# bobu36000/gym-chess

Hardware: AMD Instinct MI355X
Metric: env steps/sec at 65 536 boards per GPU (random-policy self-play to terminal, auto-reset) (higher is better)
Workload: dtype u64

## Files before the change

### gym-chess_amd/csrc/gc_host_env.h

```cpp
#pragma once

static bool srv_enabled() {
    static const bool off = getenv("GC_SINGLE_SERVER") && atoi(getenv("GC_SINGLE_SERVER")) == 0;
    return !off;
}
static int srv_stop(void* p) {
    gc_env* e = static_cast<gc_env*>(p);
    return e->srv.stop(e->device, e);
}
static int srv_call(gc_env* e, int board, int op, int action, int flags) {
    return e->srv.call(
        e->device, e, srv_stop,
        [&](SrvBox* b) {
            if (e->srv.launch && e->srv_board != board && (srv_stop(e) || devsrv_claim(devsrv(e->device), e, srv_stop)))
                return -1;
            __atomic_store_n(&b->op, (u32)op, __ATOMIC_RELAXED);
            __atomic_store_n(&b->action, action, __ATOMIC_RELAXED);
            __atomic_store_n(&b->flags, (u32)flags, __ATOMIC_RELAXED);
            return 0;
        },
        [&]() -> int {
            HIPCHK(hipStreamSynchronize(e->stream));
            e->srv_board = board;
            return 0;
        },
        [&](SrvBox* box_d, u32 seq, u32 launch) {
            k_single_server<<<1, 64, 0, e->srv.stream>>>(e->d, board, box_d, e->srec_d, seq, launch);
        });
}

static int set_window_kind(gc_env* e, bool uncapped) {
    const int bits = uncapped ? HTAB_BITS_UNCAPPED : HTAB_BITS;
    if (bits != e->d.hbits) {
        size_t nb64 = ((size_t)e->n + 63) / 64 * 64;
        u64* t = nullptr;
        if (dalloc(&t, ((size_t)8 << bits) * nb64)) return -1;
        HIPCHK(hipMemsetAsync(t, 0, ((size_t)64 << bits) * nb64, e->stream));
        (void)hipFree(e->d.htab);
        e->d.htab = t;
        e->d.hbits = bits;
    }
    if (uncapped && !e->d.ic.spill.ent) {
        if (spill_alloc(e, spill_bits_for(e->n))) return -1;
    } else if (!uncapped && e->d.ic.spill.ent) {
        HIPCHK(hipStreamSynchronize(e->stream));
        spill_drop(e);
        if (spill_publish(e)) return -1;
    }
    return 0;
}

static void launch_reset(gc_env* e, const uint8_t* mask, int select) {
    if (e->rules && e->d.opp) k_fenv_reset<true><<<grid_for(e->n), BLOCK, 0, e->stream>>>(e->d, mask, select);
    else if (e->rules) k_fenv_reset<false><<<grid_for(e->n), BLOCK, 0, e->stream>>>(e->d, mask, select);
    else if (e->d.opp) k_env_reset<true><<<grid_for(e->n), BLOCK, 0, e->stream>>>(e->d, mask, select);
    else k_env_reset<false><<<grid_for(e->n), BLOCK, 0, e->stream>>>(e->d, mask, select);
}
template <bool POLICY>
static void launch_step(gc_env* e) {
    if (e->rules && e->d.opp) k_fenv_step<POLICY, true><<<grid_for(e->n), BLOCK, 0, e->stream>>>(e->d);
    else if (e->rules) k_fenv_step<POLICY, false><<<grid_for(e->n), BLOCK, 0, e->stream>>>(e->d);
    else if (e->d.opp) k_env_step<POLICY, true><<<grid_for(e->n), BLOCK, 0, e->stream>>>(e->d);
    else k_env_step<POLICY, false><<<grid_for(e->n), BLOCK, 0, e->stream>>>(e->d);
}

struct ResetInfo {
    const EnvDev::InitCache* icd;
    const uint16_t* racts;
    u32 rinfo;
};
static ResetInfo reset_info(const gc_env* e) {
    const EnvDev::InitCache& ic = e->rules ? e->ic_f : e->d.ic;
    return ResetInfo{e->rules ? e->icd_f : e->icd, e->rules ? e->racts_f : e->d.reset_acts,
                     (ic.table ? 1u << 16 : 0u) | (u32)(ic.total & 0xFFFF)};
}

static const uint16_t* sw_table(const ResetInfo& r) {
    return r.racts ? r.racts + RESET_ACTS_MAX : r.racts;
}
static bool pair_ok(const gc_env* e) {
    if (!e->d.opp) return true;
    if (e->rules) return false;
    const EnvDev::InitCache& ic = e->d.ic;
    return ic.usable && ic.table && (!e->d.agent_black || ic.open_safe);
}
static int pair_opp(const gc_env* e) { return e->d.opp ? (e->d.agent_black ? 2 : 1) : 0; }

static_assert(PAIR_BOARDS == QUAD_BOARDS, "one board block size");
struct LaunchGeom {
    dim3 grid, block;
};
static int board_blocks(const gc_env* e) { return (e->n + PAIR_BOARDS - 1) / PAIR_BOARDS; }
static LaunchGeom pair_geom(int nb) { return {dim3((nb + PAIRS_WG - 1) / PAIRS_WG), dim3(2 * PAIR_BOARDS * PAIRS_WG)}; }
static LaunchGeom quad_geom(int nb) { return {dim3((nb + QUADS_WG - 1) / QUADS_WG), dim3(4 * QUAD_BOARDS * QUADS_WG)}; }

template <class K>
static K pair_variant(const gc_env* e, K fide, K none, K vs_white, K vs_black) {
    if (e->rules) return fide;
    const int opp = pair_opp(e);
    return opp == 0 ? none : opp == 1 ? vs_white : vs_black;
}
static const uint16_t* pair_racts(const gc_env* e, const ResetInfo& r) { return e->rules ? r.racts : sw_table(r); }

static void launch_step2(gc_env* e, hipStream_t st, int b0 = 0, int nb = -1) {
    const EnvDev& d = e->d;
    const ResetInfo r = reset_info(e);
    const LaunchGeom g = pair_geom(nb < 0 ? board_blocks(e) : nb);
    const auto kernel = pair_variant(e, k_env_step2<true>, k_env_step2<false>, k_env_step2<false, 1>, k_env_step2<false, 2>);
    kernel<<<g.grid, g.block, 0, st>>>(e->slab, d.n, b0, d.seed, d.htab, pair_racts(e, r), r.icd, r.rinfo);
}

extern "C" int gc_env_create(int device, int n_boards, uint64_t seed, const int8_t* initial_board, gc_env** out) {
    if (!out) return fail("null out pointer");
    if (n_boards <= 0) return fail("n_boards must be > 0");
    int nd = 0;
    HIPCHK(hipGetDeviceCount(&nd));
    if (device < 0 || device >= nd) return fail("device index out of range");
    static const int8_t DEF[64] = {-3, -5, -4, -2, -1, -4, -5, -3, -6, -6, -6, -6, -6, -6, -6, -6,
                                   0,  0,  0,  0,  0,  0,  0,  0,  0,  0,  0,  0,  0,  0,  0,  0,
                                   0,  0,  0,  0,  0,  0,  0,  0,  0,  0,  0,  0,  0,  0,  0,  0,
                                   6,  6,  6,  6,  6,  6,  6,  6,  3,  5,  4,  2,  1,  4,  5,  3};
    const int8_t* ib = initial_board ? initial_board : DEF;
    if (check_boards(1, ib)) return -1;
    gc_env* e = new gc_env();
    e->device = device;
    e->n = n_boards;
    e->seed = seed;
    int n = n_boards;
    size_t nb64 = ((size_t)n + 63) / 64 * 64;
    hipError_t he = hipSetDevice(device);
    if (he == hipSuccess) he = hipStreamCreateWithFlags(&e->stream, hipStreamNonBlocking);
    if (he != hipSuccess) { env_free(e); delete e; return fail(std::string("stream: ") + hipGetErrorString(he)); }
    if (dalloc(&e->slab, Slab::BYTES_PER_BOARD * (size_t)n) ||
        dalloc(&e->d.htab, (size_t)HTAB * 8 * nb64) || dalloc(&e->mbox, (size_t)64 * n) ||
        dalloc(&e->m8, (size_t)8 * n) || dalloc(&e->mask, n) || dalloc(&e->counts, n) || dalloc(&e->stats, (size_t)8 * n + 8) ) {
        std::string m = g_err;
        env_free(e); delete e;
        return fail(m);
    }
    {
        uint8_t* sl = e->slab;
        size_t nz = (size_t)n;
        e->bb = reinterpret_cast<u64*>(sl);
        e->meta = reinterpret_cast<u32*>(sl + Slab::meta(nz));
        e->d.hgen = reinterpret_cast<u32*>(sl + Slab::hgen(nz));
        e->d.draw = reinterpret_cast<u32*>(sl + Slab::draw(nz));
        e->d.nsteps = reinterpret_cast<u32*>(sl + Slab::nsteps(nz));
        e->d.reward = reinterpret_cast<int32_t*>(sl + Slab::reward(nz));
        e->d.act = reinterpret_cast<uint16_t*>(sl + Slab::act(nz));
        e->d.done = sl + Slab::done(nz);
        e->d.reason = sl + Slab::reason(nz);
    }
    Pos ip = from_mailbox(ib, 0);
    u64 ibb[NBB] = {ip.k, ip.q, ip.r, ip.b, ip.n, ip.p, ip.w};
    for (int j = 0; j < NBB; j++) e->d.init[j] = ibb[j];
    he = hipSuccess;
    if (he == hipSuccess) he = hipMemsetAsync(e->d.draw, 0, (size_t)4 * n, e->stream);
    if (he == hipSuccess) he = hipMemsetAsync(e->d.htab, 0, (size_t)64 * HTAB * nb64, e->stream);
    if (he == hipSuccess) he = hipMemsetAsync(e->d.hgen, 0, (size_t)4 * n, e->stream);
    if (he == hipSuccess) he = hipMemsetAsync(e->d.nsteps, 0, (size_t)4 * n, e->stream);
    if (he == hipSuccess) he = hipMemsetAsync(e->d.reward, 0, (size_t)4 * n, e->stream);
    if (he == hipSuccess) he = hipMemsetAsync(e->d.done, 0, (size_t)n, e->stream);
    if (he == hipSuccess) he = hipMemsetAsync(e->d.reason, 0, (size_t)n, e->stream);
    if (he == hipSuccess) he = hipMemsetAsync(e->stats, 0, (size_t)64 * n, e->stream);
    for (auto& v : e->ev) if (he == hipSuccess) he = hipEventCreate(&v);
    if (he != hipSuccess) { env_free(e); delete e; return fail(std::string("env init: ") + hipGetErrorString(he)); }
    e->d.st = SoA{e->bb, e->meta, n};
    e->d.seed = seed;
    e->d.n = n;
    e->d.opp = 0;
    e->d.agent_black = 0;
    e->d.hbits = HTAB_BITS;
    {
        EnvDev::InitCache* dic = nullptr;
        uint16_t* dacts = nullptr;
        if (dalloc(&dic, 1) || dalloc(&dacts, 2 * RESET_ACTS_MAX)) {
            std::string m = g_err; (void)hipFree(dic); env_free(e); delete e; return fail(m);
// ... 344 lines not shown
    if (kind < 0 || kind > 3) return fail("kind: 0 h2h, 1 h2d, 2 d2h, 3 d2d");
    HIPCHK(hipSetDevice(e->device));
    HIPCHK(hipMemcpyAsync(dst, src, bytes, (hipMemcpyKind)kind, e->stream));
    HIPCHK(hipStreamSynchronize(e->stream));
    return 0;
}

static int issue_plies(gc_env* e, int n) {
    if (e->n_sub <= 1) {
        for (int p = 0; p < n; p++) launch_step2(e, e->stream);
        HIPCHK(hipGetLastError());
        return 0;
    }
    const int blocks = board_blocks(e);
    const int k = e->n_sub < blocks ? e->n_sub : blocks;
    const int per = ((blocks + k - 1) / k + PAIRS_WG - 1) / PAIRS_WG * PAIRS_WG;
    HIPCHK(hipEventRecord(e->fork_ev, e->stream));
    for (int j = 0; j < k; j++) HIPCHK(hipStreamWaitEvent(e->sub[j], e->fork_ev, 0));
    for (int p = 0; p < n; p++)
        for (int j = 0; j < k; j++) {
            int b0 = j * per, nb = blocks - b0 < per ? blocks - b0 : per;
            if (nb > 0) launch_step2(e, e->sub[j], b0, nb);
        }
    HIPCHK(hipGetLastError());
    for (int j = 0; j < k; j++) {
        HIPCHK(hipEventRecord(e->sub_ev[j], e->sub[j]));
        HIPCHK(hipStreamWaitEvent(e->stream, e->sub_ev[j], 0));
    }
    return 0;
}

static int step_random(gc_env* e, int n_plies) {
    if (pair_ok(e)) return n_plies > 0 ? issue_plies(e, n_plies) : 0;
    for (int p = 0; p < n_plies; p++) {
        launch_step<true>(e);
        HIPCHK(hipGetLastError());
    }
    return 0;
}
extern "C" int gc_env_step_random(gc_env* e, int n_plies) {
    if (!e) return fail("null env");
    SRV_QUIESCE(e);
    if (!e->policy_ready) return fail("policy actions stale: call gc_env_reset or gc_env_select_random first");
    HIPCHK(hipSetDevice(e->device));
    if (spill_before(e)) return -1;
    for (int p = 0; p < n_plies;) {
        const int k = spill_chunk(e, n_plies - p);
        if (k < 0 || step_random(e, k)) return -1;
        p += k;
    }
    return spill_after(e);
}

extern "C" int gc_env_set_streams(gc_env* e, int k) {
    if (!e) return fail("null env");
    if (k < 1 || k > GC_MAX_SUBSTREAMS) return fail("streams must be in [1, 8]");
    HIPCHK(hipSetDevice(e->device));
    for (int j = 0; j < k; j++) {
        if (!e->sub[j]) HIPCHK(hipStreamCreateWithFlags(&e->sub[j], hipStreamNonBlocking));
        if (!e->sub_ev[j]) HIPCHK(hipEventCreateWithFlags(&e->sub_ev[j], hipEventDisableTiming));
    }
    if (!e->fork_ev) HIPCHK(hipEventCreateWithFlags(&e->fork_ev, hipEventDisableTiming));
    e->n_sub = k;
    return 0;
}

extern "C" int gc_env_paired(gc_env* e) {
    if (!e) return fail("null env");
    return pair_ok(e) ? 1 : 0;
}

static bool use_quad(const gc_env* e) {
    static const bool no_quad = getenv("GC_NO_QUAD") != nullptr;
    return !no_quad && !e->rules && pair_opp(e) == 0 && e->d.ic.table;
}

static int occ_min_plies() {
    static const int v = getenv("GC_OCC_MIN_PLIES") ? atoi(getenv("GC_OCC_MIN_PLIES")) : 600;
    return v;
}

extern "C" int gc_env_rollout_occ_min_plies(void) { return occ_min_plies(); }

extern "C" int gc_env_rollout_waves(gc_env* e) {
    if (!e) return fail("null env");
    return pair_ok(e) ? (use_quad(e) ? 4 : 2) : 1;
}

extern "C" int gc_env_select_random(gc_env* e) {
    if (!e) return fail("null env");
    SRV_QUIESCE(e);
    HIPCHK(hipSetDevice(e->device));
    if (e->rules) k_fenv_select<<<grid_for(e->n), BLOCK, 0, e->stream>>>(e->d);
    else k_select<<<grid_for(e->n), BLOCK, 0, e->stream>>>(e->d);
    HIPCHK(hipGetLastError());
    e->policy_ready = true;
    return 0;
}

static int issue_rollout(gc_env* e, int n_plies, uint64_t* d_trace, bool stats) {
    uint64_t* const st = stats ? e->stats : nullptr;
    const bool pair = pair_ok(e);
    const EnvDev& d = e->d;
    const ResetInfo r = reset_info(e);
    const LaunchGeom pg = pair_geom(board_blocks(e)), qg = quad_geom(board_blocks(e));
    for (int p0 = 0, k = 0; p0 < n_plies; p0 += k) {
        k = spill_chunk(e, n_plies - p0 < ROLLOUT_MAX_PLIES ? n_plies - p0 : ROLLOUT_MAX_PLIES);
        if (k < 0) return -1;
        u64* tr = d_trace ? reinterpret_cast<u64*>(d_trace) + (size_t)p0 * e->n : nullptr;
        const u32 ri = r.rinfo | ((u32)k << 18);
        e->done_expect = 0;
        if (pair && use_quad(e)) {
            const auto kernel = k >= occ_min_plies() ? k_env_rollout4<true> : k_env_rollout4<false>;
            kernel<<<qg.grid, qg.block, 0, e->stream>>>(e->slab, d.n, d.seed, d.htab, sw_table(r), r.icd, ri, st, tr);
            e->done_expect = ++e->done_issued;
        } else if (pair) {
            const auto kernel = pair_variant(e, k_env_rollout2<true>, k_env_rollout2<false>, k_env_rollout2<false, 1>,
                                             k_env_rollout2<false, 2>);
            kernel<<<pg.grid, pg.block, 0, e->stream>>>(e->slab, d.n, d.seed, d.htab, pair_racts(e, r), r.icd, ri, st, tr);
        } else if (e->rules) {
            k_fenv_rollout<true><<<grid_for(e->n), BLOCK, 0, e->stream>>>(e->d, k, tr, st);
        } else if (e->d.opp) {
            k_env_rollout<true><<<grid_for(e->n), BLOCK, 0, e->stream>>>(e->d, k, tr, st);
        } else {
            k_env_rollout<false><<<grid_for(e->n), BLOCK, 0, e->stream>>>(e->d, k, tr, st);
        }
        hipError_t le = hipGetLastError();
        if (le != hipSuccess) return fail(std::string("rollout launch: ") + hipGetErrorString(le));
    }
    return 0;
}

extern "C" int gc_env_rollout(gc_env* e, int n_plies, int16_t* tr_action, int16_t* tr_reward, uint8_t* tr_done,
                              uint8_t* tr_reason, uint64_t* stats8) {
    if (!e) return fail("null env");
    SRV_QUIESCE(e);
    if (n_plies < 0) return fail("n_plies must be >= 0");
    if (!e->policy_ready) return fail("policy actions stale: call gc_env_reset or gc_env_select_random first");
    HIPCHK(hipSetDevice(e->device));
    const bool trace = tr_action || tr_reward || tr_done || tr_reason;
    const size_t cnt = (size_t)n_plies * e->n;
    Temps tmps;
    u64* dt = nullptr;
    if (trace && cnt && tmps.alloc(&dt, cnt)) return -1;
    if (spill_before(e)) return -1;
    HIPCHK(hipMemsetAsync(e->stats, 0, (size_t)64 * e->n, e->stream));
    if (issue_rollout(e, n_plies, dt, true) || spill_after(e)) return -1;
    if (trace && cnt) {
        std::vector<u64> h(cnt);
        hipError_t ce = hipMemcpyAsync(h.data(), dt, cnt * 8, hipMemcpyDeviceToHost, e->stream);
        if (ce == hipSuccess) ce = hipStreamSynchronize(e->stream);
        if (ce != hipSuccess) return fail(std::string("rollout trace: ") + hipGetErrorString(ce));
        for (size_t t = 0; t < cnt; t++) {
            const u64 w = h[t];
            if (tr_action) tr_action[t] = (int16_t)(uint16_t)w;
            if (tr_reward) tr_reward[t] = (int16_t)(uint16_t)(w >> 16);
            if (tr_done) tr_done[t] = (uint8_t)(w >> 32);
            if (tr_reason) tr_reason[t] = (uint8_t)(w >> 40);
        }
    }
    if (stats8) {
        uint64_t* sums = e->stats + (size_t)8 * e->n;
        HIPCHK(hipMemsetAsync(sums, 0, 64, e->stream));
        k_sum_stats<<<grid_for(e->n), BLOCK, 0, e->stream>>>(e->stats, e->n, reinterpret_cast<unsigned long long*>(sums));
        HIPCHK(hipGetLastError());
        HIPCHK(hipMemcpyAsync(stats8, sums, 64, hipMemcpyDeviceToHost, e->stream));
        HIPCHK(hipStreamSynchronize(e->stream));
    }
    return 0;
}

extern "C" int gc_env_rollout_device(gc_env* e, int n_plies, uint64_t* d_trace, int ev_begin, int ev_end) {
    if (!e) return fail("null env");
    SRV_QUIESCE(e);
    if (n_plies < 0) return fail("n_plies must be >= 0");
    if (ev_begin < -1 || ev_begin >= 8 || ev_end < -1 || ev_end >= 8) return fail("event slots: -1 or 0..7");
    if (!e->policy_ready) return fail("policy actions stale: call gc_env_reset or gc_env_select_random first");
    HIPCHK(hipSetDevice(e->device));
    if (spill_before(e)) return -1;
    if (ev_begin >= 0) HIPCHK(hipEventRecord(e->ev[ev_begin], e->stream));
    if (issue_rollout(e, n_plies, d_trace, false)) return -1;
    if (ev_end >= 0) HIPCHK(hipEventRecord(e->ev[ev_end], e->stream));
    return spill_after(e);
}

extern "C" int gc_env_get_outputs(gc_env* e, int32_t* reward, uint8_t* done, uint8_t* reason, uint16_t* next_action,
                                  uint32_t* nsteps) {
    if (!e) return fail("null env");
    SRV_QUIESCE(e);
    HIPCHK(hipSetDevice(e->device));
    if (reward) HIPCHK(hipMemcpyAsync(reward, e->d.reward, (size_t)4 * e->n, hipMemcpyDeviceToHost, e->stream));
    if (done) HIPCHK(hipMemcpyAsync(done, e->d.done, e->n, hipMemcpyDeviceToHost, e->stream));
    if (reason) HIPCHK(hipMemcpyAsync(reason, e->d.reason, e->n, hipMemcpyDeviceToHost, e->stream));
    if (next_action) HIPCHK(hipMemcpyAsync(next_action, e->d.act, (size_t)2 * e->n, hipMemcpyDeviceToHost, e->stream));
    if (nsteps) HIPCHK(hipMemcpyAsync(nsteps, e->d.nsteps, (size_t)4 * e->n, hipMemcpyDeviceToHost, e->stream));
    HIPCHK(hipStreamSynchronize(e->stream));
// ... 83 lines not shown
    if (!e || !mask) return fail("null argument");
    SRV_QUIESCE(e);
    HIPCHK(hipSetDevice(e->device));
    if (!e->lmask && dalloc(&e->lmask, (size_t)65 * e->n)) return -1;
    if (e->rules) k_fmask<<<grid_for(e->n), BLOCK, 0, e->stream>>>(e->d.st, e->lmask, e->counts);
    else k_mask<<<grid_for(e->n), BLOCK, 0, e->stream>>>(e->d.st, e->lmask, e->counts);
    HIPCHK(hipGetLastError());
    HIPCHK(hipMemcpyAsync(mask, e->lmask, (size_t)8 * 65 * e->n, hipMemcpyDeviceToHost, e->stream));
    if (counts) HIPCHK(hipMemcpyAsync(counts, e->counts, (size_t)4 * e->n, hipMemcpyDeviceToHost, e->stream));
    HIPCHK(hipStreamSynchronize(e->stream));
    return 0;
}

extern "C" int gc_env_synchronize(gc_env* e) {
    if (!e) return fail("null env");
    HIPCHK(hipSetDevice(e->device));
    static const long spin_us = getenv("GC_SPIN_US") ? atol(getenv("GC_SPIN_US")) : 20000;
    if (spin_us > 0) {
        const auto t0 = std::chrono::steady_clock::now();
        for (;;) {
            const hipError_t q = hipStreamQuery(e->stream);
            if (q == hipSuccess) return 0;
            if (q != hipErrorNotReady) return fail(std::string("stream: ") + hipGetErrorString(q));
            if (std::chrono::steady_clock::now() - t0 > std::chrono::microseconds(spin_us)) break;
        }
    }
    HIPCHK(hipStreamSynchronize(e->stream));
    return 0;
}

extern "C" int gc_env_wait_rollout(gc_env* e) {
    if (!e) return fail("null env");
    if (!e->done_expect || !e->done_host) return gc_env_synchronize(e);
    const u32 want = e->done_expect;
    for (unsigned k = 0;; k++) {
        if ((int)(__atomic_load_n(e->done_host, __ATOMIC_ACQUIRE) - want) >= 0) return 0;
        if ((k & 255) == 255) {
            const hipError_t q = hipStreamQuery(e->stream);
            if (q == hipSuccess) return 0;
            if (q != hipErrorNotReady) return fail(std::string("stream: ") + hipGetErrorString(q));
        }
    }
}

extern "C" int gc_env_record_event(gc_env* e, int slot) {
    if (!e || slot < 0 || slot >= 8) return fail("bad env or event slot");
    HIPCHK(hipEventRecord(e->ev[slot], e->stream));
    return 0;
}

extern "C" int gc_env_elapsed_ms(gc_env* e, int a, int b, float* ms) {
    if (!e || !ms || a < 0 || a >= 8 || b < 0 || b >= 8) return fail("bad argument");
    HIPCHK(hipEventSynchronize(e->ev[b]));
    HIPCHK(hipEventElapsedTime(ms, e->ev[a], e->ev[b]));
    return 0;
}

__global__ void k_window_sum(SoA st, unsigned long long* out) {
    int i = blockIdx.x * blockDim.x + threadIdx.x;
    unsigned long long v = i < st.n ? (unsigned long long)hl_of(st.meta[i]) : 0ull;
    for (int o = 32; o > 0; o >>= 1) v += __shfl_down(v, o, 64);
    if ((threadIdx.x & 63) == 0 && v) atomicAdd(out, v);
}

extern "C" int gc_env_window_sum(gc_env* e, uint64_t* sum) {
    if (!e || !sum) return fail("null argument");
    SRV_QUIESCE(e);
    HIPCHK(hipSetDevice(e->device));
    Temps tmps;
    unsigned long long* d = nullptr;
    if (tmps.alloc(&d, 1)) return -1;
    HIPCHK(hipMemsetAsync(d, 0, 8, e->stream));
    k_window_sum<<<grid_for(e->n), BLOCK, 0, e->stream>>>(e->d.st, d);
    HIPCHK(hipGetLastError());
    HIPCHK(hipMemcpyAsync(sum, d, 8, hipMemcpyDeviceToHost, e->stream));
    HIPCHK(hipStreamSynchronize(e->stream));
    return 0;
}

#ifdef GC_PSTAMPS
extern "C" int gc_debug_pstamps(gc_env* e, int n_plies, uint64_t* out ) {
    Temps tmps;
    unsigned long long* d = nullptr;
    const LaunchGeom g = use_quad(e) ? quad_geom(board_blocks(e)) : pair_geom(board_blocks(e));
    const size_t waves = (size_t)g.grid.x * (g.block.x / 64);
    if (tmps.alloc(&d, waves * 12)) return -1;
    HIPCHK(hipMemsetAsync(d, 0, waves * 96, e->stream));
    HIPCHK(hipStreamSynchronize(e->stream));
    HIPCHK(hipMemcpyToSymbol(HIP_SYMBOL(g_pst_out), &d, sizeof(d)));
    if (issue_rollout(e, n_plies, nullptr, false)) return -1;
    HIPCHK(hipMemcpyAsync(out, d, waves * 96, hipMemcpyDeviceToHost, e->stream));
    HIPCHK(hipStreamSynchronize(e->stream));
    unsigned long long* z = nullptr;
    HIPCHK(hipMemcpyToSymbol(HIP_SYMBOL(g_pst_out), &z, sizeof(z)));
    return 0;
}
#endif

#ifdef GC_PSTAMPS
static unsigned long long* g_api_pst = nullptr;
extern "C" int gc_debug_api_pstamps(gc_env* e, int on, uint64_t* out ) {
    const LaunchGeom g = quad_geom(board_blocks(e));
    const size_t waves = (size_t)g.grid.x * (g.block.x / 64);
    HIPCHK(hipStreamSynchronize(e->stream));
    if (on) {
        if (!g_api_pst && dalloc(&g_api_pst, waves * 12)) return -1;
        HIPCHK(hipMemset(g_api_pst, 0, waves * 96));
        HIPCHK(hipMemcpyToSymbol(HIP_SYMBOL(g_pst_out), &g_api_pst, sizeof(g_api_pst)));
        return 0;
    }
    if (g_api_pst && out) HIPCHK(hipMemcpy(out, g_api_pst, waves * 96, hipMemcpyDeviceToHost));
    unsigned long long* z = nullptr;
    HIPCHK(hipMemcpyToSymbol(HIP_SYMBOL(g_pst_out), &z, sizeof(z)));
    return 0;
}
#endif

#ifdef GC_STAMPS
extern "C" int gc_debug_stamps(gc_env* e, int n_plies, uint64_t* out ) {
    Temps tmps;
    unsigned long long* d = nullptr;
    size_t cnt = (size_t)((e->n + 63) / 64) * 16;
    if (tmps.alloc(&d, cnt)) return -1;
    HIPCHK(hipMemsetAsync(d, 0, cnt * 8, e->stream));
    HIPCHK(hipStreamSynchronize(e->stream));
    HIPCHK(hipMemcpyToSymbol(HIP_SYMBOL(g_stamp_out), &d, sizeof(d)));
    for (int p = 0; p < n_plies; p++) {
        launch_step2(e, e->stream);
    }
    HIPCHK(hipGetLastError());
    HIPCHK(hipMemcpyAsync(out, d, cnt * 8, hipMemcpyDeviceToHost, e->stream));
    HIPCHK(hipStreamSynchronize(e->stream));
    unsigned long long* z = nullptr;
    HIPCHK(hipMemcpyToSymbol(HIP_SYMBOL(g_stamp_out), &z, sizeof(z)));
    return 0;
}
#endif

__global__ void k_get_ep(SoA st, int8_t* __restrict__ files) {
    int i = blockIdx.x * blockDim.x + threadIdx.x;
    if (i >= st.n) return;
    u32 m = st.meta[i];
    files[i] = (m & gcf::M_EP) ? (int8_t)((m & gcf::M_EP_MASK) >> gcf::M_EP_SHIFT) : (int8_t)-1;
}
__global__ void k_set_ep(SoA st, const int8_t* __restrict__ files) {
    int i = blockIdx.x * blockDim.x + threadIdx.x;
    if (i >= st.n) return;
    st.meta[i] = gcf::with_ep(st.meta[i], files[i] < 0 ? -1 : (int)files[i]);
}

extern "C" int gc_env_get_en_passant(gc_env* e, int8_t* files) {
    if (!e || !files) return fail("null argument");
    HIPCHK(hipSetDevice(e->device));
    if (!e->ep && dalloc(&e->ep, e->n)) return -1;
    k_get_ep<<<grid_for(e->n), BLOCK, 0, e->stream>>>(e->d.st, e->ep);
    HIPCHK(hipGetLastError());
    HIPCHK(hipMemcpyAsync(files, e->ep, e->n, hipMemcpyDeviceToHost, e->stream));
    HIPCHK(hipStreamSynchronize(e->stream));
    return 0;
}

extern "C" int gc_env_set_en_passant(gc_env* e, const int8_t* files) {
    if (!e || !files) return fail("null argument");
    for (int i = 0; i < e->n; i++) {
        if (files[i] > 7) return fail("en-passant file out of range at index " + std::to_string(i));
        if (files[i] >= 0 && !e->rules) return fail("en passant exists only under rules=fide (Q3: the reference has none)");
    }
// ... 17 lines not shown
```

### gym-chess_amd/csrc/gymchess.hip

```cpp
#include <hip/hip_runtime.h>
#include <hipcub/hipcub.hpp>

#include <cmath>
#include <cstdio>
#include <cstdlib>
#include <cstring>
#include <atomic>
#include <chrono>
#include <mutex>
#include <string>
#include <type_traits>
#include <vector>

#ifdef GC_STAMPS
__shared__ unsigned long long gc_stamp_lds[4][8];
__device__ __forceinline__ void gc_stamp(int k) {
    __builtin_amdgcn_sched_barrier(0);
    unsigned long long t;
#ifdef GC_STAMPS_REAL
    asm volatile("s_memrealtime %0\n\ts_waitcnt lgkmcnt(0)" : "=s"(t)::"memory");
    if (k == 0) {
        unsigned hw, xcc;
        asm volatile("s_getreg_b32 %0, hwreg(HW_REG_HW_ID)\n\ts_getreg_b32 %1, hwreg(HW_REG_XCC_ID)"
                     : "=s"(hw), "=s"(xcc));
// ... 1661 lines not shown
    PAIR_PROLOGUE
    uint64_t steps = 0, rsum = 0;
    u32 e_mate = 0, e_rep = 0, e_cap = 0, e_nomove = 0, e_err = 0;
    StepOut o = {0, 0, R_NONE, 0};
#ifdef GC_PSTAMPS
    unsigned long long rt0 = 0, rt1 = 0;
    if (l == 0) {
        for (int k = 0; k < 8; k++) gc_pst[threadIdx.x >> 6][k] = 0;
        gc_pst[threadIdx.x >> 6][8] = __builtin_amdgcn_s_memtime();
    }
    rt0 = __builtin_amdgcn_s_memrealtime();
#endif
    const int wg_half = ((nn + PAIR_BOARDS * PAIRS_WG - 1) / (PAIR_BOARDS * PAIRS_WG)) >> 1;
    auto plies_loop = [&](auto R, auto ST) {
        for (int p = 0; p < plies; p++) {
            int played = a;
            if (GC_PAIR_FAIR) {
                if ((((int)blockIdx.x >= wg_half) ? 1 : 0) ^ (p & 1)) __builtin_amdgcn_s_setprio(1);
                else __builtin_amdgcn_s_setprio(0);
            }
            o = pair_step<OPP, true, FIDE>(Ls, L, C, R, l, i, live, rp, s, a, d, h, nst);
#ifdef GC_PSTAMPS
            if (p == 0) rt1 = __builtin_amdgcn_s_memrealtime();
#endif
            if (R) {
                if (trace && live) trace[(size_t)p * nn + i] = trace_word(played == A_NONE ? -1 : played, o);
                if (!ST) {
                } else if (played == A_NONE) {
                    e_nomove++;
                } else {
                    steps++;
                    rsum += (uint64_t)(int64_t)o.reward;
                    if (o.done) {
                        e_mate += o.reason == R_MATE || o.reason == R_MATED;
                        e_rep += o.reason == R_REPETITION;
                        e_cap += o.reason == R_MOVE_CAP;
                        e_err += o.reason == R_BOTH_CHECKED || o.reason == R_WINDOW_FULL;
                        e_nomove += o.reason == R_OPP_NO_MOVE;
                    }
                }
                h.commit();
            }
        }
#ifdef GC_PSTAMPS
        if (g_pst_out != nullptr && l == 0) {
            const size_t w = (size_t)blockIdx.x * (blockDim.x >> 6) + (threadIdx.x >> 6);
            for (int k = 0; k < 8; k++) g_pst_out[w * 12 + k] = gc_pst[threadIdx.x >> 6][k];
            g_pst_out[w * 12 + 8] = g_pst_entry;
            g_pst_out[w * 12 + 9] = rt0;
            g_pst_out[w * 12 + 10] = rt1;
            g_pst_out[w * 12 + 11] = __builtin_amdgcn_s_memrealtime();
        }
#endif
        const PairIO io = store_io(slab, nn);
        if (live) {
            if (R == 0) {
                io.act[i] = (uint16_t)a;
                io.draw[i] = d;
            } else {
                io.store(i, s);
                h.flush(g0);
                io.nsteps[i] = nst;
                io.reward[i] = o.reward;
                io.done[i] = (uint8_t)o.done;
                io.reason[i] = (uint8_t)o.reason;
                if (ST) {
                    uint64_t* so = stats + 8 * (size_t)i;
                    so[0] += steps; so[1] += rsum;
                    so[2 + R_MATE] += e_mate; so[2 + R_REPETITION] += e_rep; so[2 + R_MOVE_CAP] += e_cap;
                    so[2 + R_NO_MOVES] += e_nomove; so[2 + R_BOTH_CHECKED] += e_err;
                }
            }
        }
    };
    if (role == 0) plies_loop(RoleC<0>{}, std::false_type{});
    else if (stats) plies_loop(RoleC<1>{}, std::true_type{});
    else plies_loop(RoleC<1>{}, std::false_type{});
}

#define QUAD_BOARDS 64
#ifndef QUADS_WG
#define QUADS_WG 2
#endif

struct QuadLds {
    u64 sets[SW_SETS][QUAD_BOARDS];
    u64 ns[NBB][QUAD_BOARDS];
    u32 nmeta[QUAD_BOARDS];
    int32_t mr[QUAD_BOARDS];
    u32 irrev[QUAD_BOARDS];
    u64 pin3[3][QUAD_BOARDS];
    u32 f0[QUAD_BOARDS];
    u64 enemy[3][QUAD_BOARDS];
    u32 f1[QUAD_BOARDS];
    u64 cwx[2][4][QUAD_BOARDS];
    u64 cw0[2][QUAD_BOARDS];
    u32 part[4][QUAD_BOARDS];
    u32 rep[QUAD_BOARDS];
    u32 x0[QUAD_BOARDS];
    u32 ra[QUAD_BOARDS];
    u32 act[QUAD_BOARDS];
    u32 pick[QUAD_BOARDS];
    u32 castles[QUAD_BOARDS];
    u64 occ[HTAB / 64][QUAD_BOARDS];
    u32 nkey[QUAD_BOARDS];
    u32 rkey0;
    Pos rp;
};
template <class LT>
struct QuadSetsT {
    LT& L;
    int l;
    u64 cw[4];
    int part;
    __device__ void put(int j, u64 t) {
        L.sets[j][l] = t;
        const int c = popc(t);
        cw[j >> 3] |= (u64)c << (8 * (j & 7));
        part += c;
    }
    template <int LO, int HI>
    __device__ void put_all(const u64* t) {
#pragma unroll
        for (int j = LO; j < HI; j++) put(j, t[j - LO]);
    }
};
using QuadSets = QuadSetsT<QuadLds>;

struct QuadPend {
    bool pending;
    bool have;
    uint16_t ra;
    __device__ int resolve(const QuadLds& L, int l, int a) const {
        return !pending ? a : have ? (int)L.pick[l] : (int)ra;
    }
};

struct OccQ {
    bool valid;
    bool clr;
    bool probe;
    bool fast;
};
#ifndef GC_WG_FAIR
#define GC_WG_FAIR 1
#endif
#define QSETPRIO(x, up)                                       \
    do {                                                      \
        if (GC_WG_FAIR && (up)) __builtin_amdgcn_s_setprio((x) + 1); \
        else __builtin_amdgcn_s_setprio(x);                   \
    } while (0)
template <int R, bool OCC>
__device__ __forceinline__ StepOut quad_ply(QuadLds& L, const PairCtx& C, int l, int i, bool live, Pos& s, int& a,
                                            u32& d, DevHist& h, u32& nst, RepProbe& pr, QuadPend& pend, OccQ& oq,
                                            bool up = false) {
    constexpr bool CARRY = R < 2;
    if (R == 0) QSETPRIO(2, up);
    if (R == 2) QSETPRIO(0, up);
    if (GC_WG_FAIR && R == 1) QSETPRIO(2, up);
    if (GC_WG_FAIR && R == 3) QSETPRIO(0, up);
    if (R == 0) a = pend.resolve(L, l, a);
    u32 x0 = 0;
    uint16_t ra = (uint16_t)A_NONE;
    if (R == 1) {
        x0 = philox_x0(C.seed, (u32)i, d);
        if (C.rtable) ra = C.racts[scale_rank(x0, C.rtotal)];
// ... 137 lines not shown
    }
    if (R == 0) L.part[0][l] = (u32)Q.part;
    PST(4);
    pair_barrier();
    PST(5);
    StepOut o = {0, 0, R_NONE, 0};
    if (R == 0) QSETPRIO(0, up);
    if (R == 2) QSETPRIO(2, up);
    if (R == 2) {
        const int total = (int)L.part[0][l] + Q.part + (int)L.part[3][l];
        u64 cw[4];
#pragma unroll
        for (int k = 0; k < 4; k++) cw[k] = Q.cw[k] | L.cwx[1][k][l];
        cw[0] |= L.cw0[0][l];
        cw[1] |= L.cw0[1][l];
        g.castles = L.castles[l];
        L.pick[l] = total > 0 ? (u32)sw_pick_lds(L, l, g, cw, total, (int)scale_rank(L.x0[l], (u32)total)) : (u32)A_NONE;
    }
    if constexpr (CARRY) {
        const int total = gen ? (R == 0 ? Q.part : (int)L.part[0][l]) + (int)L.part[2][l] + (int)L.part[3][l] : 0;
        if (R == 0) {
            const u32 rpk = L.rep[l];
            c = (int)(rpk & 0xFFu);
            hl = rpk >> 8;
            ra = (uint16_t)L.ra[l];
        } else {
            h.commit();
        }
        bool have = false;
        if (none) {
            o.reason = R_NO_MOVES;
        } else {
            nst += 1;
            if (done0) { o.done = 1; o.reason = R_DONE_ALREADY; }
            else if (cap) { o.done = 1; o.reason = R_MOVE_CAP; }
            else if (both) { o.done = 1; o.reason = R_BOTH_CHECKED; }
            else {
                const u32 chk = white ? ((my_chk ? M_WCHK : 0u) | (opp_chk ? M_BCHK : 0u))
                                      : ((opp_chk ? M_WCHK : 0u) | (my_chk ? M_BCHK : 0u));
                s = ns;
                s.meta = with_hl((ns.meta & ~(u32)(M_WCHK | M_BCHK | M_DONE)) | chk | ((c >= 3 || c == 0) ? M_DONE : 0u), hl);
                o.reward = -10 + mr;
                o.moved = 1;
                if (c >= 3) { o.done = 1; o.reason = R_REPETITION; }
                if (c == 0) { o.done = 1; o.reason = R_WINDOW_FULL; }
                if (total == 0 && opp_chk) {
                    s.meta |= M_DONE;
                    o.done = 1;
                    o.reward += 100;
                    o.reason = R_MATE;
                }
                if (!o.done && !white) s.meta += (1u << M_MC_SHIFT);
                have = true;
            }
            if (o.done) have = false;
        }
        if (!have) {
            s = L.rp;
            h.bump_gen();
        }
        if (R == 1 && OCC) {
            pr.key = have ? L.nkey[l] : L.rkey0;
            if (!have) {
                oq.valid = true;
                oq.clr = true;
            }
            oq.fast = !(live && have && oq.probe);
            const ulonglong2* src = oq.fast ? reinterpret_cast<const ulonglong2*>(C.icd)
                                            : reinterpret_cast<const ulonglong2*>(h.htab + h.entry((int)(pr.key & (HTAB - 1))) * 8);
            const ulonglong2 e0 = src[0], e1 = src[1], e2 = src[2], e3 = src[3];
            pr.e0 = RepEntry{e0.x, e0.y, e1.x, e1.y, e2.x, e2.y, e3.x, e3.y};
        } else if (R == 1 && live) {
            rep_prefetch(h, s, pr);
        }
        const int tot = have ? total : (int)C.rtotal;
        d += tot > 0 ? 1u : 0u;
        if (R == 0) pend = QuadPend{true, have, ra};
    }
    PST(6);
    pair_barrier();
    return o;
}

__shared__ QuadLds g_quad_lds[QUADS_WG];

template <int RR, bool ST, bool OCC>
__device__ __forceinline__ void quad_run(uint8_t* __restrict__ slab, int nn, uint64_t seed, u64* __restrict__ htab,
                                      const uint16_t* __restrict__ racts, const EnvDev::InitCache* __restrict__ icd,
                                      u32 rinfo, int plies, uint64_t* __restrict__ stats, u64* __restrict__ trace,
                                      int qw, int l, int i) {
    QuadLds& L = g_quad_lds[qw];
    const bool live = i < nn;
    const int ii = live ? i : nn - 1;
    const PairIO in_io(slab, nn);
    const PairCtx C = {seed, htab, in_io.hgen, racts, icd, (rinfo >> 16) != 0, rinfo & 0xFFFFu};
    Pos s{};
    u32 ua = 0, g0 = 0, nst = 0, d = 0;
    if (RR < 2) {
        s = in_io.load(ii);
        ua = in_io.act[ii];
        g0 = in_io.hgen[ii];
        nst = in_io.nsteps[ii];
        d = in_io.draw[ii];
        pin(s); pin(ua); pin(g0); pin(nst); pin(d);
    }
    if (RR == 3 && l == 0) {
        const Pos rp = icd->pos;
        L.rp = rp;
        if (OCC) L.rkey0 = board_key(rp);
    }
    int a = (int)ua;
    DevHist h = DevHist{htab, in_io.hgen, g0, ii, HTAB_BITS};
    RepProbe pr;
    if (RR == 1 && live) rep_prefetch(h, s, pr);
    OccQ oq{RR == 1 && hl_of(s.meta) == 0, RR == 1, true, false};
    QuadPend pend{false, false, 0};
    const int wg_half = ((nn + QUAD_BOARDS * QUADS_WG - 1) / (QUAD_BOARDS * QUADS_WG)) >> 1;
#ifdef GC_PSTAMPS
    const unsigned long long g_pst_entry = pst_entry_where();
    unsigned long long rt1 = 0;
    if (l == 0) {
        for (int k = 0; k < 8; k++) gc_pst[threadIdx.x >> 6][k] = 0;
        gc_pst[threadIdx.x >> 6][8] = __builtin_amdgcn_s_memtime();
    }
    const unsigned long long rt0 = __builtin_amdgcn_s_memrealtime();
#endif
    u32 sa = 0, sb = 0, sc = 0;
    int32_t rsum = 0;
    StepOut o = {0, 0, R_NONE, 0};
    for (int p = 0; p < plies; p++) {
#ifndef GC_TURN_SHIFT
#define GC_TURN_SHIFT 2
#endif
        const bool up = GC_WG_FAIR && ((((int)blockIdx.x >= wg_half) ? 1 : 0) ^ ((p >> GC_TURN_SHIFT) & 1));
        o = quad_ply<RR, OCC>(L, C, l, i, live, s, a, d, h, nst, pr, pend, oq, up);
        const int played = a;
#ifdef GC_PSTAMPS
        if (p == 0) rt1 = __builtin_amdgcn_s_memrealtime();
#endif
        if (RR == 1) {
            if (trace && live) trace[(size_t)p * nn + i] = trace_word(played == A_NONE ? -1 : played, o);
            if (!ST) {
            } else if (played == A_NONE) {
                sc += 1u << 16;
            } else {
                sa += 1u;
                rsum += o.reward;
                if (o.done) {
                    sb += (o.reason == R_MATE || o.reason == R_MATED ? 1u : 0u) | (o.reason == R_REPETITION ? 1u << 16 : 0u);
                    sc += (o.reason == R_MOVE_CAP ? 1u : 0u) | (o.reason == R_OPP_NO_MOVE ? 1u << 16 : 0u);
                    sa += o.reason == R_BOTH_CHECKED || o.reason == R_WINDOW_FULL ? 1u << 16 : 0u;
                }
            }
            h.commit();
        }
    }
#ifdef GC_PSTAMPS
    if (g_pst_out != nullptr && l == 0) {
        const size_t w = (size_t)blockIdx.x * (blockDim.x >> 6) + (threadIdx.x >> 6);
        for (int k = 0; k < 8; k++) g_pst_out[w * 12 + k] = gc_pst[threadIdx.x >> 6][k];
        g_pst_out[w * 12 + 8] = g_pst_entry;
        g_pst_out[w * 12 + 9] = rt0;
        g_pst_out[w * 12 + 10] = rt1;
        g_pst_out[w * 12 + 11] = __builtin_amdgcn_s_memrealtime();
    }
#endif
    if (!live || RR >= 2) return;
    const PairIO io = store_io(slab, nn);
    if (RR == 0) {
        a = pend.resolve(L, l, a);
        io.act[i] = (uint16_t)a;
        io.draw[i] = d;
    } else {
        io.store(i, s);
        if (h.gen() != g0) io.hgen[i] = h.gen();
        io.nsteps[i] = nst;
        io.reward[i] = o.reward;
        io.done[i] = (uint8_t)o.done;
        io.reason[i] = (uint8_t)o.reason;
        if (ST) {
            uint64_t* so = stats + 8 * (size_t)i;
            so[0] += sa & 0xFFFFu; so[1] += (uint64_t)(int64_t)rsum;
            so[2 + R_MATE] += sb & 0xFFFFu; so[2 + R_REPETITION] += sb >> 16; so[2 + R_MOVE_CAP] += sc & 0xFFFFu;
            so[2 + R_NO_MOVES] += sc >> 16; so[2 + R_BOTH_CHECKED] += sa >> 16;
        }
    }
}

template <bool OCC>
__global__ void __launch_bounds__(4 * QUAD_BOARDS * QUADS_WG) __attribute__((amdgpu_waves_per_eu(4)))
    k_env_rollout4(uint8_t* __restrict__ slab, int nn, uint64_t seed, u64* __restrict__ htab,
                   const uint16_t* __restrict__ racts, const EnvDev::InitCache* __restrict__ icd, u32 rinfo,
                   uint64_t* __restrict__ stats, u64* __restrict__ trace) {
    const int plies = (int)(rinfo >> 18);
    rinfo &= 0x1FFFFu;
    const int wv = __builtin_amdgcn_readfirstlane((int)(threadIdx.x >> 6));
    const int qw = wv >> 2;
#ifndef GC_QXOR
#define GC_QXOR 2
#endif
    const int role = (wv & 3) ^ ((qw & 1) ? GC_QXOR : 0);
    const int l = threadIdx.x & (QUAD_BOARDS - 1);
    const int i = (blockIdx.x * QUADS_WG + qw) * QUAD_BOARDS + l;
#ifndef GC_QPRIO
#define GC_QPRIO 0x0A
#endif
    switch ((GC_QPRIO >> (2 * role)) & 3) {
        case 1: __builtin_amdgcn_s_setprio(1); break;
        case 2: __builtin_amdgcn_s_setprio(2); break;
        case 3: __builtin_amdgcn_s_setprio(3); break;
        default: break;
    }
    switch (role) {
        case 0: quad_run<0, false, OCC>(slab, nn, seed, htab, racts, icd, rinfo, plies, stats, trace, qw, l, i); break;
        case 1:
            if (stats) quad_run<1, true, OCC>(slab, nn, seed, htab, racts, icd, rinfo, plies, stats, trace, qw, l, i);
            else quad_run<1, false, OCC>(slab, nn, seed, htab, racts, icd, rinfo, plies, stats, trace, qw, l, i);
            break;
        case 2: quad_run<2, false, OCC>(slab, nn, seed, htab, racts, icd, rinfo, plies, stats, trace, qw, l, i); break;
        default: quad_run<3, false, OCC>(slab, nn, seed, htab, racts, icd, rinfo, plies, stats, trace, qw, l, i); break;
    }
    const EnvDev::InitCache::DoneWord dw = icd->done;
    if (dw.ctr) {
        __syncthreads();
        if (threadIdx.x == 0) {
            const u32 prev = __hip_atomic_fetch_add(dw.ctr, 1u, __ATOMIC_RELAXED, __HIP_MEMORY_SCOPE_AGENT);
            const u32 wgs = (u32)(nn + QUAD_BOARDS * QUADS_WG - 1) / (QUAD_BOARDS * QUADS_WG);
            if (prev == wgs - 1) {
                __hip_atomic_store(dw.ctr, 0u, __ATOMIC_RELAXED, __HIP_MEMORY_SCOPE_AGENT);
                const u32 v = __hip_atomic_fetch_add(dw.seq, 1u, __ATOMIC_RELAXED, __HIP_MEMORY_SCOPE_AGENT) + 1u;
                __hip_atomic_store(dw.host, v, __ATOMIC_RELAXED, __HIP_MEMORY_SCOPE_SYSTEM);
            }
        }
    }
}

template <bool OPP>
__global__ void __launch_bounds__(BLOCK) k_env_rollout(EnvDev e, int plies, u64* trace, uint64_t* stats) {
    LDS_SCRATCH_DECL;
    int i = blockIdx.x * blockDim.x + threadIdx.x;
    if (i >= e.n) return;
    Pos s = e.st.load(i);
    u32 g0 = e.hgen[i], d = e.draw[i], ua = e.act[i];
    pin(s); pin(g0); pin(d); pin(ua);
    DevHist h = e.hist(i, g0);
    PolicyCtx pc = {e.seed, (u32)i, d};
    int a = (int)ua;
    uint64_t steps = 0, rsum = 0;
    u32 e_mate = 0, e_rep = 0, e_cap = 0, e_nomove = 0, e_err = 0;
    StepOut o = {0, 0, R_NONE, 0};
    for (int p = 0; p < plies; p++) {
        o = {0, 0, R_NONE, 0};
        Gen g;
        MoveSet ms;
        bool have = false;
        int played = a;
        if (a == A_NONE) {
            reset_board(e, s, h);
            o.reason = R_NO_MOVES;
            e_nomove++;
            played = -1;
        } else {
            o = OPP ? env_step_vs<false>(s, h, a, nullptr, g, ms, scr, pc) : env_step<false>(s, h, a, nullptr, g, ms, scr);
            have = o.moved;
            steps++;
            rsum += (uint64_t)(int64_t)o.reward;
            if (o.done) {
                e_mate += o.reason == R_MATE || o.reason == R_MATED;
                e_rep += o.reason == R_REPETITION;
                e_cap += o.reason == R_MOVE_CAP;
                e_err += o.reason == R_BOTH_CHECKED || o.reason == R_WINDOW_FULL;
                e_nomove += o.reason == R_OPP_NO_MOVE;
                reset_board(e, s, h);
                have = false;
            }
        }
        if (OPP && !have) after_reset<OPP>(e, s, h, g, ms, scr, pc);
        if (trace) trace[(size_t)p * e.n + i] = trace_word(played, o);
        a = selfplay_pick(s, pc);
        h.commit();
    }
    e.reward[i] = o.reward;
    e.done[i] = (uint8_t)o.done;
    e.reason[i] = (uint8_t)o.reason;
    e.st.store(i, s);
    h.flush(g0);
    e.draw[i] = pc.draw;
    e.act[i] = (uint16_t)a;
    e.nsteps[i] += (u32)steps;
    if (stats) {
        uint64_t* so = stats + 8 * (size_t)i;
        so[0] += steps; so[1] += rsum;
        so[2 + R_MATE] += e_mate; so[2 + R_REPETITION] += e_rep; so[2 + R_MOVE_CAP] += e_cap;
        so[2 + R_NO_MOVES] += e_nomove; so[2 + R_BOTH_CHECKED] += e_err;
    }
}

enum { SOP_RESET = 0, SOP_AGENT = 1, SOP_REPLY = 2, SOP_OPEN = 3, SOP_SYNC = 4, SOP_SET = 5 };
static_assert(sizeof(gc_single_record) == 728, "gym_chess_amd.single._REC mirrors this layout");
struct SingleCtx {
    Pos s;
    Gen g;
    DevHist h;
    u32 g0;
    int status, reward, done, reason, chk, pend, white, flags, op, has_g;
    int cached;
    unsigned long long t[3];
};
enum { SPEND_NONE = 0, SPEND_AGENT = 1, SPEND_REPLY = 2 };

__device__ __noinline__ void single_begin(const EnvDev& e, int i, int op, int action, int flags, int valid,
// ... 1732 lines not shown
```

Measured before the change: 17.32 billion.

## Launch single-quad workgroups for long rollouts with four-way fairness rotation

Result: faster. 18.11 billion, median of 6 (+4.6%).

```diff
diff --git a/gym-chess_amd/csrc/gc_host_env.h b/gym-chess_amd/csrc/gc_host_env.h
--- a/gym-chess_amd/csrc/gc_host_env.h
+++ b/gym-chess_amd/csrc/gc_host_env.h
@@ -93,6 +93,7 @@
 static int board_blocks(const gc_env* e) { return (e->n + PAIR_BOARDS - 1) / PAIR_BOARDS; }
 static LaunchGeom pair_geom(int nb) { return {dim3((nb + PAIRS_WG - 1) / PAIRS_WG), dim3(2 * PAIR_BOARDS * PAIRS_WG)}; }
 static LaunchGeom quad_geom(int nb) { return {dim3((nb + QUADS_WG - 1) / QUADS_WG), dim3(4 * QUAD_BOARDS * QUADS_WG)}; }
+static LaunchGeom roll_geom(int nb, int qw) { return {dim3((nb + qw - 1) / qw), dim3(4 * QUAD_BOARDS * qw)}; }
 
 template <class K>
 static K pair_variant(const gc_env* e, K fide, K none, K vs_white, K vs_black) {
@@ -603,6 +604,9 @@
 
 extern "C" int gc_env_rollout_occ_min_plies(void) { return occ_min_plies(); }
 
+#define ROLL_SPLIT_MIN_PLIES 50
+static int roll_quads_wg(int plies) { return plies >= ROLL_SPLIT_MIN_PLIES ? ROLL_QUADS_WG : QUADS_WG; }
+
 extern "C" int gc_env_rollout_waves(gc_env* e) {
     if (!e) return fail("null env");
     return pair_ok(e) ? (use_quad(e) ? 4 : 2) : 1;
@@ -624,7 +628,7 @@
     const bool pair = pair_ok(e);
     const EnvDev& d = e->d;
     const ResetInfo r = reset_info(e);
-    const LaunchGeom pg = pair_geom(board_blocks(e)), qg = quad_geom(board_blocks(e));
+    const LaunchGeom pg = pair_geom(board_blocks(e));
     for (int p0 = 0, k = 0; p0 < n_plies; p0 += k) {
         k = spill_chunk(e, n_plies - p0 < ROLLOUT_MAX_PLIES ? n_plies - p0 : ROLLOUT_MAX_PLIES);
         if (k < 0) return -1;
@@ -632,7 +636,10 @@
         const u32 ri = r.rinfo | ((u32)k << 18);
         e->done_expect = 0;
         if (pair && use_quad(e)) {
-            const auto kernel = k >= occ_min_plies() ? k_env_rollout4<true> : k_env_rollout4<false>;
+            const bool occ = k >= occ_min_plies(), split = roll_quads_wg(k) == ROLL_QUADS_WG;
+            const LaunchGeom qg = roll_geom(board_blocks(e), roll_quads_wg(k));
+            const auto kernel = split ? (occ ? k_env_rollout4<true, ROLL_QUADS_WG> : k_env_rollout4<false, ROLL_QUADS_WG>)
+                                      : (occ ? k_env_rollout4<true, QUADS_WG> : k_env_rollout4<false, QUADS_WG>);
             kernel<<<qg.grid, qg.block, 0, e->stream>>>(e->slab, d.n, d.seed, d.htab, sw_table(r), r.icd, ri, st, tr);
             e->done_expect = ++e->done_issued;
         } else if (pair) {
@@ -882,7 +889,7 @@
 extern "C" int gc_debug_pstamps(gc_env* e, int n_plies, uint64_t* out ) {
     Temps tmps;
     unsigned long long* d = nullptr;
-    const LaunchGeom g = use_quad(e) ? quad_geom(board_blocks(e)) : pair_geom(board_blocks(e));
+    const LaunchGeom g = use_quad(e) ? roll_geom(board_blocks(e), roll_quads_wg(n_plies)) : pair_geom(board_blocks(e));
     const size_t waves = (size_t)g.grid.x * (g.block.x / 64);
     if (tmps.alloc(&d, waves * 12)) return -1;
     HIPCHK(hipMemsetAsync(d, 0, waves * 96, e->stream));
diff --git a/gym-chess_amd/csrc/gymchess.hip b/gym-chess_amd/csrc/gymchess.hip
--- a/gym-chess_amd/csrc/gymchess.hip
+++ b/gym-chess_amd/csrc/gymchess.hip
@@ -1767,6 +1767,10 @@
 #ifndef QUADS_WG
 #define QUADS_WG 2
 #endif
+#ifndef GC_QXOR
+#define GC_QXOR 2
+#endif
+#define ROLL_QUADS_WG 1
 
 struct QuadLds {
     u64 sets[SW_SETS][QUAD_BOARDS];
@@ -2070,14 +2074,32 @@
     return o;
 }
 
-__shared__ QuadLds g_quad_lds[QUADS_WG];
-
-template <int RR, bool ST, bool OCC>
+__shared__ QuadLds g_quad_lds[ROLL_QUADS_WG];
+__shared__ QuadLds g_quad_lds2[QUADS_WG];
+template <int QW>
+__device__ __forceinline__ QuadLds& roll_lds(int qw) {
+    if constexpr (QW == ROLL_QUADS_WG) return g_quad_lds[qw];
+    else return g_quad_lds2[qw];
+}
+
+#define ROLL_TURNS 0xCA69C6A9C69AC69Cull
+template <int QW>
+__device__ __forceinline__ int roll_place(int block, int wgs) {
+    const int part = wgs / (4 / QW);
+    return (part ? block / part : block) & (4 / QW - 1);
+}
+template <int QW>
+__device__ __forceinline__ bool roll_turn(int place, int turn) {
+    if (QW == 2) return ((place ^ turn) & 1) != 0;
+    return ((ROLL_TURNS >> (4 * (turn & 15) + place)) & 1) != 0;
+}
+
+template <int RR, bool ST, bool OCC, int QW>
 __device__ __forceinline__ void quad_run(uint8_t* __restrict__ slab, int nn, uint64_t seed, u64* __restrict__ htab,
                                       const uint16_t* __restrict__ racts, const EnvDev::InitCache* __restrict__ icd,
                                       u32 rinfo, int plies, uint64_t* __restrict__ stats, u64* __restrict__ trace,
-                                      int qw, int l, int i) {
-    QuadLds& L = g_quad_lds[qw];
+                                      int qw, int l, int i, int place) {
+    QuadLds& L = roll_lds<QW>(qw);
     const bool live = i < nn;
     const int ii = live ? i : nn - 1;
     const PairIO in_io(slab, nn);
@@ -2103,7 +2125,6 @@
     if (RR == 1 && live) rep_prefetch(h, s, pr);
     OccQ oq{RR == 1 && hl_of(s.meta) == 0, RR == 1, true, false};
     QuadPend pend{false, false, 0};
-    const int wg_half = ((nn + QUAD_BOARDS * QUADS_WG - 1) / (QUAD_BOARDS * QUADS_WG)) >> 1;
 #ifdef GC_PSTAMPS
     const unsigned long long g_pst_entry = pst_entry_where();
     unsigned long long rt1 = 0;
@@ -2120,7 +2141,7 @@
 #ifndef GC_TURN_SHIFT
 #define GC_TURN_SHIFT 2
 #endif
-        const bool up = GC_WG_FAIR && ((((int)blockIdx.x >= wg_half) ? 1 : 0) ^ ((p >> GC_TURN_SHIFT) & 1));
+        const bool up = GC_WG_FAIR && roll_turn<QW>(place, p >> GC_TURN_SHIFT);
         o = quad_ply<RR, OCC>(L, C, l, i, live, s, a, d, h, nst, pr, pend, oq, up);
         const int played = a;
 #ifdef GC_PSTAMPS
@@ -2175,8 +2196,8 @@
     }
 }
 
-template <bool OCC>
-__global__ void __launch_bounds__(4 * QUAD_BOARDS * QUADS_WG) __attribute__((amdgpu_waves_per_eu(4)))
+template <bool OCC, int QW>
+__global__ void __launch_bounds__(4 * QUAD_BOARDS * QW) __attribute__((amdgpu_waves_per_eu(4)))
     k_env_rollout4(uint8_t* __restrict__ slab, int nn, uint64_t seed, u64* __restrict__ htab,
                    const uint16_t* __restrict__ racts, const EnvDev::InitCache* __restrict__ icd, u32 rinfo,
                    uint64_t* __restrict__ stats, u64* __restrict__ trace) {
@@ -2184,12 +2205,11 @@
     rinfo &= 0x1FFFFu;
     const int wv = __builtin_amdgcn_readfirstlane((int)(threadIdx.x >> 6));
     const int qw = wv >> 2;
-#ifndef GC_QXOR
-#define GC_QXOR 2
-#endif
+    const int wgs = (nn + QUAD_BOARDS * QW - 1) / (QUAD_BOARDS * QW);
+    const int place = roll_place<QW>((int)blockIdx.x, wgs);
     const int role = (wv & 3) ^ ((qw & 1) ? GC_QXOR : 0);
     const int l = threadIdx.x & (QUAD_BOARDS - 1);
-    const int i = (blockIdx.x * QUADS_WG + qw) * QUAD_BOARDS + l;
+    const int i = (blockIdx.x * QW + qw) * QUAD_BOARDS + l;
 #ifndef GC_QPRIO
 #define GC_QPRIO 0x0A
 #endif
@@ -2200,21 +2220,20 @@
         default: break;
     }
     switch (role) {
-        case 0: quad_run<0, false, OCC>(slab, nn, seed, htab, racts, icd, rinfo, plies, stats, trace, qw, l, i); break;
+        case 0: quad_run<0, false, OCC, QW>(slab, nn, seed, htab, racts, icd, rinfo, plies, stats, trace, qw, l, i, place); break;
         case 1:
-            if (stats) quad_run<1, true, OCC>(slab, nn, seed, htab, racts, icd, rinfo, plies, stats, trace, qw, l, i);
-            else quad_run<1, false, OCC>(slab, nn, seed, htab, racts, icd, rinfo, plies, stats, trace, qw, l, i);
+            if (stats) quad_run<1, true, OCC, QW>(slab, nn, seed, htab, racts, icd, rinfo, plies, stats, trace, qw, l, i, place);
+            else quad_run<1, false, OCC, QW>(slab, nn, seed, htab, racts, icd, rinfo, plies, stats, trace, qw, l, i, place);
             break;
-        case 2: quad_run<2, false, OCC>(slab, nn, seed, htab, racts, icd, rinfo, plies, stats, trace, qw, l, i); break;
-        default: quad_run<3, false, OCC>(slab, nn, seed, htab, racts, icd, rinfo, plies, stats, trace, qw, l, i); break;
+        case 2: quad_run<2, false, OCC, QW>(slab, nn, seed, htab, racts, icd, rinfo, plies, stats, trace, qw, l, i, place); break;
+        default: quad_run<3, false, OCC, QW>(slab, nn, seed, htab, racts, icd, rinfo, plies, stats, trace, qw, l, i, place); break;
     }
     const EnvDev::InitCache::DoneWord dw = icd->done;
     if (dw.ctr) {
         __syncthreads();
         if (threadIdx.x == 0) {
             const u32 prev = __hip_atomic_fetch_add(dw.ctr, 1u, __ATOMIC_RELAXED, __HIP_MEMORY_SCOPE_AGENT);
-            const u32 wgs = (u32)(nn + QUAD_BOARDS * QUADS_WG - 1) / (QUAD_BOARDS * QUADS_WG);
-            if (prev == wgs - 1) {
+            if (prev == (u32)wgs - 1) {
                 __hip_atomic_store(dw.ctr, 0u, __ATOMIC_RELAXED, __HIP_MEMORY_SCOPE_AGENT);
                 const u32 v = __hip_atomic_fetch_add(dw.seq, 1u, __ATOMIC_RELAXED, __HIP_MEMORY_SCOPE_AGENT) + 1u;
                 __hip_atomic_store(dw.host, v, __ATOMIC_RELAXED, __HIP_MEMORY_SCOPE_SYSTEM);
```
